# criteo-research/reco-gym

Measured on AMD Instinct MI355X. Metric: env steps/sec (organic+bandit events emitted/sec), reco-gym-v1 P=10000 K=20, higher is better.
Workload: dtype f64 (state, click, transition, policy, propensities); organic logits on MFMA as a 2-way fp16 split of fp32 operands (fp32 accumulate), every index certified against f64; 1 GPU; c3: reco-gym-v1 P=10000 K=20 sigma_omega=0.0 policy=ouc; users_per_gpu=10000000, users_total=10000000, log=16 B/row device log + float64 ps side array

## Files before the change

### recogym_amd/csrc/rg_common.hpp

```cpp

#include <hip/hip_runtime.h>

#include <cmath>
#include <cstdarg>
#include <cstdio>
#include <cstdlib>
#include <cstring>
#include <new>
#include <utility>
#include <vector>

#include "../../include/recogym_hip.h"
#include "../../include/recogym_rng.h"

#pragma once

#ifndef RG_WALK_PRECISE_CHUNK
#define RG_WALK_PRECISE_CHUNK 1
#endif

namespace rgk {

constexpr uint32_t kMaxSteps = 1u << 16;
constexpr int kBlock = 256;
// ... 210 lines not shown
    Switches w;
    const auto rd = [](const char* name) { Switch s; if (const char* e = getenv(name)) { s.set = true; s.c0 = e[0]; s.num = atoi(e); } return s; };
#define RG_SWITCH_READ(f, name) w.f = rd("RECOGYM_" name);
    RG_SWITCHES(RG_SWITCH_READ)
#undef RG_SWITCH_READ
    const char* const draws[] = {"", "f64", "fp32", "bf16", "f16"};
    if (const char* e = getenv("RECOGYM_DRAW")) for (int i = 1; i < 5; ++i) if (!strcmp(e, draws[i])) w.draw = static_cast<Switches::Draw>(i);
    if (const char* e = getenv("RECOGYM_BF16")) w.bf16_lean = !strcmp(e, "lean");
    if (const char* e = getenv("RECOGYM_REPACK_MIN")) w.repack_min = static_cast<uint64_t>(strtoull(e, nullptr, 10));
    return w;
}

struct RunOpts {
    int exact_tile;
    int exact_mix;
    int slices;
    int sweep_prefix_off;
    int debug;
    unsigned long long repack_min;
};

#define RG_LEDGER_FAMILIES(X) \
    X(draw_f64) X(draw_fp32) X(draw16_fused) X(draw16_sliced) X(search) X(draw_tp) X(pick) X(draw_cached) \
    X(sweep_xh) X(exact_m) X(exact_tile) X(exact_h) X(walk) X(walk2) X(walk_solo) \
    X(advance) X(advance_run) X(tail) X(repack) X(env0) X(logreg_screen) X(logreg_acts) X(logreg_sample) X(logreg_poly) \
    X(logreg_poly_w) X(sort_tiled) X(sort_plain) X(bayes_vb)
struct Ledger {
#define RG_LEDGER_FIELD(f) uint64_t f = 0;
    RG_LEDGER_FAMILIES(RG_LEDGER_FIELD)
#undef RG_LEDGER_FIELD
};

enum ProfClass { kProfSweep, kProfSearch , kProfResolve , kProfLogreg, kProfAdvance,
                 kProfWalk1, kProfWalk2 , kProfTail, kProfNone  };

struct WhTable {
    const double* tab;
    uint32_t n;
    uint32_t f32;
};

struct WhRun {
    WhTable wt;
    unsigned long long* rows;
    uint32_t* spill;
    uint32_t spill_cap;
};
// ... 4 lines not shown
    DevSim d;
    WhRun wh;
    RunOpts opt;
    void* workspace;
    size_t workspace_bytes;
    uint32_t t;
    uint32_t run_ahead;
    uint32_t lr_part_rows;
    uint32_t live_upper;
    bool tables_set, users_reset;
    bool repacked;
    bool walk;
    int walk_occ;
    bool walk2;
    bool walk_solo;
    int n_cus;
    int pipe_groups;
    int pipe_occ1, pipe_occ2;
    int pipe_xblocks;
    bool fin_in_sweep;
    uint32_t pipe_min_users;
    double prof_pipe_ms;
    uint32_t fate_base; const unsigned long long* fate_count;
    uint32_t repack_every;
    bool sort_plain;
    uint32_t tail_below;
    uint32_t* h_pinned;
    char* h_step;
    size_t mfma_smem, bf16_smem;
    void (*bf16_kernel)(DevSim, uint32_t, uint32_t);
    void (*xh_kernel)(DevSim, uint32_t, uint32_t);
    size_t xh_smem;
    int xh_waves;
    void (*tp_kernel)(DevSim, uint32_t, uint32_t);
    void (*pick_kernel)(DevSim, uint32_t, uint32_t);
    size_t tp_smem;
    uint32_t tp_nts;
    uint32_t sweep_lds;
    bool handover_auto;
    uint32_t draw_threads, draw_users;
    bool profiling;
    std::vector<hipEvent_t> prof_events;
    std::vector<ProfClass> prof_cls;
    size_t prof_used;
    double prof_ms[kProfNone];
    uint64_t prof_launches;
// ... 36 lines not shown
search_kernel_t logreg_acts_kernel();
search_kernel_t logreg_screen_kernel();
search_kernel_t logreg_decide_kernel();
search_kernel_t logreg_sample_kernel();
search_kernel_t poly_acts_kernel();
void (*poly_debug_kernel())(DevSim, int32_t*, uint8_t*);
search_kernel_t bayes_acts_kernel();
void (*bayes_debug_kernel())(DevSim, int32_t*, uint8_t*, double*);
void (*wh_insert_kernel())(DevSim, WhRun, uint32_t);
void (*wh_acts_kernel())(DevSim, WhRun, uint32_t, uint32_t);
void (*wh_debug_set_kernel())(DevSim, WhRun, const uint32_t*, const uint32_t*, const uint16_t*, uint32_t);
void (*wh_debug_acts_kernel())(DevSim, WhRun, const uint16_t*, int32_t*, uint8_t*, uint32_t*, uint32_t*, uint32_t*, uint32_t);
constexpr int kWhGridBlocks = 512;
advance_kernel_t advance_kernel(bool eg);
advance_run_kernel_t advance_run_kernel(bool eg);
round_rows_kernel_t round_rows_kernel();
search_kernel_t tail_kernel(bool eg);
walk_kernel_t walk_kernel_for(const DevSim& d, int occ);
walk_kernel_t walk2_kernel_for(const DevSim& d, int occ);
typedef void (*solo_kernel_t)(DevSim, uint32_t, uint32_t, uint32_t);
solo_kernel_t solo_kernel_for(const DevSim& d);
void (*cache_prefix_kernel())(DevSim, int);
void (*exact_prefix_kernel())(DevSim, uint32_t);

struct Carve {
    size_t off = 0;
    char* base;
    explicit Carve(void* b) : base(static_cast<char*>(b)) {}
    template <class T> T* take(size_t n) {
        off = align_up(off, 256);
        T* p = base ? reinterpret_cast<T*>(base + off) : nullptr;
        off += n * sizeof(T);
        return p;
    }
};

constexpr uint32_t kMaxSC = 32;
constexpr uint32_t kAhatGrid = 64;
constexpr uint32_t kHoleCode = 0xFFFFFFFFu;
#ifdef RG_WALK_TIMING
#define RG_WALK_ABL(bit) (d.ablate & (1u << (bit)))
#else
#define RG_WALK_ABL(bit) (false)
#endif

constexpr int kCntTailRows = 16, kCntTailOrganic = 17, kCntTailBandit = 18, kCntTailMaxT = 19, kCntTailTicket = 20,
              kCntTailLimit = 21, kCntWalkTicket = 22, kCntParkCnt = 23;
constexpr int kCntWalkHits = RG_CNT_MEMO_HITS;
constexpr uint32_t kMaxWalkWaves = 4096;
constexpr uint32_t kParkSlack = 2u * 64u * kMaxWalkWaves;
constexpr uint32_t kWalkCtlWords = 16;

struct Geom { uint32_t KH, KS, TP, P_pad, n_chunks, sc_chunks, n_sc, N1, N2, N3, RS, TPB, F16, XNH, XNL, XRS; bool cache, all_f64, repack, tp; };

inline bool tp_class_exists(const Geom& g) { return (g.F16 == 1 && g.KH <= 10 && g.n_chunks / 4 <= kTpBins) || g.F16 == 2; }

inline Geom geom_of(const rg_config& c, uint64_t n, const Switches& sw) {
    Geom g{};
    g.all_f64 = sw.draw == Switches::kDrawF64 || sw.force_exact.is('1');
    g.repack = n >= sw.repack_min;
    const uint32_t need = (c.K + 1) / 2;
    const uint32_t opts[] = {4, 10, 16, 32, 64};
    for (uint32_t o : opts) if (!g.KH && need <= o) g.KH = o;
    if (!g.KH) { g.all_f64 = true; return g; }
    g.KS = 2 * g.KH;
    while (g.KS % 4 != 2) ++g.KS;
    g.TP = 256;
    while (g.TP > 64 && static_cast<size_t>(g.TP) * g.KS * 4 > 24 * 1024) g.TP /= 2;
    g.P_pad = static_cast<uint32_t>(align_up(c.num_products, 256)) + 256;
    g.n_chunks = (c.num_products + 31) / 32;
    g.n_chunks = (g.n_chunks + 3) & ~3u;
    {
        const uint32_t cls[][3] = {{1, 1, 1}, {2, 1, 1}, {3, 2, 1}, {4, 3, 2}, {6, 4, 2}, {12, 8, 4}};
        for (const auto& c3 : cls)
// ... 1442 lines not shown
```

### recogym_amd/csrc/rg_host.hip

```cpp

#include "rg_common.hpp"

#ifndef RG_TP_SMEM_PAD
#define RG_TP_SMEM_PAD 0
#endif
namespace rgk {

__global__ void __launch_bounds__(kBlock) k_reset_users(DevSim d) {
    if (blockIdx.x == 0 && threadIdx.x == 0) {
        d.step_cnt[0] = d.n_users;
        d.step_cnt[1] = 0;
        d.log_base[0] = d.debug_row_base;
    }
    for (uint32_t i = blockIdx.x * kBlock + threadIdx.x; i < d.n_users; i += gridDim.x * kBlock) {
        const uint32_t user = static_cast<uint32_t>(d.first_user + i);
        if (d.env_kind) {
            const rg_u32x4 w = rg_draw(d.seed, user, 0u, 0u, RG_DRAW_RESET);
            d.pv0[i] = upper_bound_f64(d.e0_cdf_init, d.P, rg_uniform(w.w[0], w.w[1]));
        } else
        for (uint32_t j = 0; 2 * j < d.K; ++j) {
            double z0, z1;
            normal_pair(d.seed, user, 0u, j, RG_DRAW_RESET, &z0, &z1);
            d.omega[static_cast<size_t>(i) * d.OMS + 2 * j] = 0.0 + d.sigma0 * z0;
            if (2 * j + 1 < d.K) d.omega[static_cast<size_t>(i) * d.OMS + 2 * j + 1] = 0.0 + d.sigma0 * z1;
// ... 113 lines not shown
            if (which >= 2 * d.KH + 2) x = fabs(d.mu_o[p]) + x * (static_cast<double>(which - (2 * d.KH + 2) + 1) * 0.25);
        } else x = fabs(d.mu_o[p]);
        m = fmax(m, x);
    }
    red[threadIdx.x] = m;
    __syncthreads();
    for (int s2 = kBlock / 2; s2 > 0; s2 >>= 1) {
        if (threadIdx.x < s2) red[threadIdx.x] = fmax(red[threadIdx.x], red[threadIdx.x + s2]);
        __syncthreads();
    }
    if (threadIdx.x == 0) d.stats[which] = static_cast<float>(red[0] * (1.0 + 1e-6));
}

__global__ void k_tail_finish(DevSim d, uint32_t t0) {
    d.log_base[t0 + 1] = d.log_base[t0] + d.counters[kCntTailRows];
    d.step_cnt[2 * (t0 + 1)] = 0;
    d.step_cnt[2 * (t0 + 1) + 1] = 0;
}

__global__ void k_walk_finish(DevSim d) {
    d.step_cnt[0] = 0; d.step_cnt[1] = 0; d.step_cnt[2] = 0; d.step_cnt[3] = 0;
    d.log_base[0] = d.debug_row_base;
    d.log_base[1] = d.counters[kCntTailRows];
}

__global__ void k_totals(DevSim d, uint32_t t_now) {
    __shared__ unsigned long long so[kBlock], sb[kBlock];
    unsigned long long o = 0, b = 0;
    for (uint32_t t = threadIdx.x; t < t_now; t += kBlock) { o += d.step_cnt[2 * t]; b += d.step_cnt[2 * t + 1]; }
    so[threadIdx.x] = o; sb[threadIdx.x] = b;
    __syncthreads();
    for (int s = kBlock / 2; s > 0; s >>= 1) {
        if (threadIdx.x < s) { so[threadIdx.x] += so[threadIdx.x + s]; sb[threadIdx.x] += sb[threadIdx.x + s]; }
        __syncthreads();
    }
    if (threadIdx.x == 0) {
        d.counters[RG_CNT_ORGANIC] = so[0] + d.counters[kCntTailOrganic];
        d.counters[RG_CNT_BANDIT] = sb[0] + d.counters[kCntTailBandit];
        d.counters[RG_CNT_LIVE] = static_cast<unsigned long long>(d.step_cnt[2 * t_now]) + d.step_cnt[2 * t_now + 1];
        d.counters[RG_CNT_STEP] = max(static_cast<unsigned long long>(t_now), d.counters[kCntTailMaxT]);
        const unsigned long long rows = d.log_base[t_now];
        d.counters[RG_CNT_LOG_ROWS] = d.log ? (rows < d.log_cap ? rows : d.log_cap) : 0ull;
        d.counters[RG_CNT_LOG_DROPPED] = d.log ? (rows > d.log_cap ? rows - d.log_cap : 0ull) : 0ull;
    }
}

// ... 616 lines not shown
    if (int rc = prof_mark(sim, st, kProfAdvance)) return rc;
    if (d.run_ahead) {
        hipLaunchKernelGGL(advance_run_kernel(d.eg_on != 0u), dim3(grid_for(upper, kAdvBlock)), dim3(kAdvBlock), 0, st, d, t, d.run_ahead);
        sim->led.advance_run += 1;
    } else {
        hipLaunchKernelGGL(advance_kernel(d.eg_on != 0u), dim3(grid_for(upper, kAdvBlock)), dim3(kAdvBlock), 0, st, d, t, d_actions);
        sim->led.advance += 1;
    }
    if (d.sigma_omega != 0.0)
        hipLaunchKernelGGL(drift_kernel(), dim3(grid_for(static_cast<uint64_t>(upper) * ((d.K + 1) / 2))), dim3(kBlock), 0, st, d, t);
    if (d.run_ahead) hipLaunchKernelGGL(round_rows_kernel(), dim3(1), dim3(1), 0, st, d, t, 0u);
    if (sim->wh.wt.tab) {
        if (int rc = prof_mark(sim, st, kProfLogreg)) return rc;
        hipLaunchKernelGGL(wh_acts_kernel(), dim3(wh_grid(upper)), dim3(kBlock), 0, st, d, sim->wh, t, 1u);
    }
    HIP_TRY(hipGetLastError());
    if (int rc = prof_mark(sim, st, kProfNone)) return rc;
    if (sim->profiling) sim->prof_launches += 1;
    sim->t = t + 1;
    return RG_OK;
}

constexpr size_t kNoWall = ~static_cast<size_t>(0);
int close_run(rg_sim* sim, hipStream_t st, uint32_t t_end, size_t wall_from = kNoWall) {
    unsigned long long* h64 = reinterpret_cast<unsigned long long*>(sim->h_pinned);
    HIP_TRY(hipMemcpyAsync(h64, sim->d.counters + kCntTailLimit, sizeof(unsigned long long), hipMemcpyDeviceToHost, st));
    HIP_TRY(hipStreamSynchronize(st));
    if (sim->profiling && wall_from != kNoWall) {
        float ms = 0.f;
        HIP_TRY(hipEventElapsedTime(&ms, sim->prof_events[wall_from], sim->prof_events[sim->prof_used - 1]));
        sim->prof_pipe_ms += ms;
    }
    sim->t = t_end;
    sim->live_upper = 0;
    if (*h64) return fail(RG_ELIMIT, "more than %u steps", kMaxSteps);
    return RG_OK;
}

int walk_begin(rg_sim* sim, hipStream_t st) {
    (void)device_cus(sim);
    if (sim->d.debug_row_base)
        HIP_TRY(hipMemcpyAsync(sim->d.counters + kCntTailRows, &sim->d.debug_row_base, sizeof(unsigned long long), hipMemcpyHostToDevice, st));
    return RG_OK;
}
int walk_end(rg_sim* sim, hipStream_t st, size_t wall_from = kNoWall) {
    if (int rc = prof_mark(sim, st, kProfNone)) return rc;
    hipLaunchKernelGGL(k_walk_finish, dim3(1), dim3(1), 0, st, sim->d);
    HIP_TRY(hipGetLastError());
    if (int rc = prof_mark(sim, st, kProfNone)) return rc;
    if (sim->profiling) sim->prof_launches += 1;
    return close_run(sim, st, 1u, wall_from);
}

int run_walk(rg_sim* sim, hipStream_t st) {
    const DevSim& d = sim->d;
    if (int rc = walk_begin(sim, st)) return rc;
    sim->fate_count = nullptr;
    bool fused_prefix = false;
    if (int rc = prof_mark(sim, st, kProfSweep)) return rc;
    {
        DevSim ds = d;
        const auto [tiles_up, S] = sweep_slices(d.n_users, sim->draw_users, sim->opt.slices, d.n_sc);
        fused_prefix = sim->walk2 && S == 1 && f16_pipelined(sim) && !sim->opt.sweep_prefix_off;
        ds.sweep_only = fused_prefix ? 2u : 1u;
        const int grid = sweep_grid(sim, static_cast<uint64_t>(tiles_up) * S);
        hipLaunchKernelGGL(sim->bf16_kernel, dim3(grid), dim3(sim->draw_threads), sim->bf16_smem, st, ds, 0u, S);
        (S > 1 ? sim->led.draw16_sliced : sim->led.draw16_fused) += 1;
    }
    if (int rc = prof_mark(sim, st, kProfSearch)) return rc;
    hipLaunchKernelGGL(finalize_kernel_for(d), dim3(grid_for(d.n_users)), dim3(kBlock), 0, st, d);
    if (sim->walk2)
        hipLaunchKernelGGL(cache_prefix_kernel(), dim3(grid_for((static_cast<uint64_t>(d.n_users) + 7) / 8, kBlock / 64)), dim3(kBlock), 0, st, d,
                           fused_prefix ? 1 : 0);
    if (int rc = prof_mark(sim, st, kProfWalk1)) return rc;
    const size_t smem = sim->walk2 ? (kBlock / 64) * walk2_wave_lds(d.policy == RG_POLICY_ORGANIC_USER_COUNT)
                                   : (kBlock / 64) * walk_wave_lds(d.KH);
    const walk_kernel_t wk = sim->walk2 ? walk2_kernel_for(d, sim->walk_occ) : walk_kernel_for(d, d.KH <= 16 ? sim->walk_occ : 1);
    auto launch_walk = [&](uint32_t n_work, int round, uint32_t in_base, uint32_t out_base) {
        const int blocks = walk_blocks(n_work, d.KH <= 16 ? sim->walk_occ : 1, sim->n_cus);
        opt_in_lds(wk, smem);
        hipLaunchKernelGGL(wk, dim3(blocks), dim3(kBlock), smem, st, d, n_work, round, walk_chunk_rows(n_work, blocks), in_base, out_base);
        (sim->walk2 ? sim->led.walk2 : sim->led.walk) += 1;
    };
    launch_walk(d.n_users, 1, 0u, 0u);
    if (int rc = prof_mark(sim, st, kProfResolve)) return rc;
    unsigned long long* h64 = reinterpret_cast<unsigned long long*>(sim->h_pinned);
    HIP_TRY(hipMemcpyAsync(h64, d.counters + kCntParkCnt, sizeof(unsigned long long), hipMemcpyDeviceToHost, st));
    HIP_TRY(hipStreamSynchronize(st));
    const uint32_t n_park = static_cast<uint32_t>(*h64);
    if (sim->opt.debug) {
        unsigned long long ev2[2] = {0, 0};
        HIP_TRY(hipMemcpy(ev2, d.counters + kCntTailOrganic, sizeof(ev2), hipMemcpyDeviceToHost));
        fprintf(stderr, "[recogym] walk round 1: %llu organic + %llu bandit events, %u users parked of %u\n", ev2[0], ev2[1], n_park, d.n_users);
    }
    if (n_park) {
        const uint32_t mfma_of_8 = static_cast<uint32_t>(sim->opt.exact_mix);
        const exact_h_kernel_t kh = mfma_of_8 < 8 ? exact_h_kernel_for(d.XKB) : nullptr;
        const exact_m_kernel_t km = kh ? nullptr : exact_m_kernel_for(d.XKB);
        if (kh) {
            HIP_TRY(hipMemsetAsync(d.counters + kCntWalkTicket, 0, sizeof(unsigned long long), st));
            const uint32_t groups = (n_park + 255u) / 256u;
            const uint32_t grid = groups < 1024u ? groups : 1024u;
            hipLaunchKernelGGL(kh, dim3(grid), dim3(kBlock), exact_m_lds(d.XKB), st, d, n_park, mfma_of_8);
            sim->led.exact_h += 1;
        } else if (km) {
            launch_exact_m(km, d, n_park, 2, 1, n_park, st);
            sim->led.exact_m += 1;
        } else return fail(RG_ESTATE, "no float64 batch kernel for K = %u", d.K);
    }
    if (int rc = prof_mark(sim, st, kProfWalk2)) return rc;
    if (n_park) {
        const uint32_t base3 = (n_park + 63u) & ~63u;
// ... 47 lines not shown
        DevSim ds = dg;
        ds.sweep_only = 2u;
        ds.fin_in_sweep = dg.fin_in_sweep = sim->fin_in_sweep ? 1u : 0u;
        const uint32_t tiles_up = (n + sim->draw_users - 1) / sim->draw_users;
        if (int rc = prof_mark(sim, st, kProfSweep)) return rc;
        if (sim->xh_kernel) { hipLaunchKernelGGL(sim->xh_kernel, dim3(grid_for((n + 32u * sim->xh_waves - 1) / (32u * sim->xh_waves), 1)), dim3(64 * sim->xh_waves), sim->xh_smem, st, ds, 0u, 1u); sim->led.sweep_xh += 1; }
        else {
        hipLaunchKernelGGL(sim->bf16_kernel, dim3(sweep_grid(sim, tiles_up)), dim3(sim->draw_threads), sim->bf16_smem, st, ds, 0u, 1u);
        sim->led.draw16_fused += 1;
        }
        if (int rc = prof_mark(sim, st, kProfSearch)) return rc;
        hipLaunchKernelGGL(finalize_kernel_for(d), dim3(grid_for(n)), dim3(kBlock), 0, st, dg);
        hipLaunchKernelGGL(cache_prefix_kernel(), dim3(grid_for((static_cast<uint64_t>(n) + 7) / 8, kBlock / 64)), dim3(kBlock), 0, st, dg, 1);
    }
    {
        DevSim dw = dg;
        dw.q_ticket = ctl + 0; dw.q_park = ctl + 1; dw.q_count = nullptr;
        const int blocks = walk_blocks(n, sim->pipe_occ1, n_cus);
        if (int rc = prof_mark(sim, st, kProfWalk1)) return rc;
        hipLaunchKernelGGL(wk, dim3(blocks), dim3(kBlock), smem, st, dw, n, 1, walk_chunk_rows(n, blocks), 0u, region);
        sim->led.walk2 += 1;
    }
    {
        DevSim dx = dg;
        dx.q_ticket = ctl + 2; dx.q_count = ctl + 1; dx.list_in = region;
        const uint32_t est = n / 3 + 4096u;
        uint32_t xgrid = (n + 255u) / 256u;
        if (xgrid > static_cast<uint32_t>(sim->pipe_xblocks)) xgrid = static_cast<uint32_t>(sim->pipe_xblocks);
        if (int rc = prof_mark(sim, st, kProfResolve)) return rc;
        hipLaunchKernelGGL(kh, dim3(xgrid), dim3(kBlock), exact_m_lds(d.XKB), st, dx, n, mfma_of_8);
        sim->led.exact_h += 1;
        hipLaunchKernelGGL(exact_prefix_kernel(), dim3(grid_for(est, kBlock / 64)), dim3(kBlock), 0, st, dx, n);
        DevSim dr = dg;
        dr.q_ticket = ctl + 3; dr.q_park = ctl_last + 0; dr.q_count = ctl + 1;
        const int blocks = walk_blocks(est, sim->pipe_occ2, n_cus);
        if (int rc = prof_mark(sim, st, kProfWalk2)) return rc;
        hipLaunchKernelGGL(wk, dim3(blocks), dim3(kBlock), smem, st, dr, n, 2, walk_chunk_rows(est, blocks), region, base_solo);
        sim->led.walk2 += 1;
    }
    sim->fate_base = base_solo; sim->fate_count = ctl_last + 0;
    if (d.walk_handover) {
        DevSim dl = d;
        dl.q_ticket = ctl_last + 1; dl.q_count = ctl_last + 0;
        const SoloShape sh = solo_shape(n / 256u + 1024u, n_cus);
        hipLaunchKernelGGL(sk, dim3(sh.blocks), dim3(kBlock), 0, st, dl, n, sh.chunk_rows, base_solo);
        sim->led.walk_solo += 1;
    }
    return walk_end(sim, st, first_mark);
}


}

namespace {
void plan_config(rg_sim* s, const rg_config* cfg, uint64_t n_users, const Switches& w) {
    DevSim& d = s->d;
    d.P = cfg->num_products; d.K = cfg->K;
    d.seed = cfg->seed; d.policy_seed = cfg->policy_seed;
    d.cdf_o0 = cfg->trans_cdf[0][0]; d.cdf_o1 = cfg->trans_cdf[0][1];
    d.cdf_b0 = cfg->trans_cdf[1][0]; d.cdf_b1 = cfg->trans_cdf[1][1];
    d.sigma0 = cfg->sigma_omega_initial; d.sigma_omega = cfg->sigma_omega; d.change_omega_for_bandits = cfg->change_omega_for_bandits;
    d.policy = lists_unresolved(cfg->policy) ? RG_POLICY_LOGREG_FROZEN : cfg->policy;
    d.lr_poly = cfg->policy == RG_POLICY_LOGREG_POLY ? 1u : cfg->policy == RG_POLICY_BAYES_VB ? 2u : 0u;
    d.ouc_select_randomly = cfg->ouc_select_randomly; d.ouc_exploit_explore = cfg->ouc_exploit_explore;
    d.ouc_reverse_pop = cfg->ouc_reverse_pop; d.ouc_epsilon = cfg->ouc_epsilon;
    d.time_mode = cfg->time_mode; d.time_mu = cfg->time_mu; d.time_sigma = cfg->time_sigma; d.env_kind = cfg->env_kind;
    d.n_users = d.n_cap = static_cast<uint32_t>(n_users);
    d.grp_lo = 0; d.grp_n = d.n_users; d.list_in = 0;
    d.q_ticket = d.counters + kCntWalkTicket; d.q_park = d.counters + kCntParkCnt; d.q_count = nullptr;
    RunOpts& o = s->opt;
    o.exact_tile = w.exact_tile.set ? 1 : 0; o.sweep_prefix_off = w.sweep_prefix_off.set ? 1 : 0; o.debug = w.debug.set ? 1 : 0;
// ... 95 lines not shown
    s->walk_solo = !w.walk_solo.is('0');
    s->n_cus = 0;
    d.walk_refill = w.walk_refill.set ? w.walk_refill.u32() : 8;
    d.walk_handover = w.walk_handover.set ? w.walk_handover.u32() : 32;
    s->handover_auto = !w.walk_handover.set;
    d.walk_click_batch = w.walk_click_batch.set ? w.walk_click_batch.u32() : 8;
    d.walk_click_join = w.walk_click_join.is('0') ? 0 : 1;
    d.walk_helpers = w.walk_helpers.set && w.walk_helpers.u32() < kWalkHelpersMax ? w.walk_helpers.u32() : kWalkHelpersMax;
    d.walk_bias = !s->walk2 ? 8 : (d.walk_helpers ? 2 : 4);
    if (w.walk_bias.set) d.walk_bias = w.walk_bias.u32();
    d.walk_search_batch = s->walk2 && d.walk_helpers ? 24 : 16;
    if (w.walk_search_batch.set) d.walk_search_batch = w.walk_search_batch.u32() ? w.walk_search_batch.u32() : 1u;
}
void plan_pipe(rg_sim* s, const Switches& w) {
    const auto in = [](const Switch& x, int lo, int hi) { return x.set && x.num >= lo && x.num <= hi; };
    s->pipe_groups = in(w.pipe, 0, 1) ? w.pipe.num : 1;
    s->pipe_occ1 = in(w.pipe_occ1, 1, s->walk_occ) ? w.pipe_occ1.num : s->walk_occ;
    s->pipe_occ2 = in(w.pipe_occ2, 1, s->walk_occ) ? w.pipe_occ2.num : s->walk_occ;
    s->pipe_xblocks = in(w.pipe_xblocks, 1, INT_MAX) ? w.pipe_xblocks.num : 1024;
    s->pipe_min_users = in(w.pipe_min, 256, INT_MAX) ? static_cast<uint32_t>(w.pipe_min.num) : 1u << 17;
    s->fin_in_sweep = !w.fin_in_sweep.is('0');
    s->d.fin_in_sweep = 0;
    s->fate_base = 0; s->fate_count = nullptr;
}
void plan_logreg_run_ahead(rg_sim* s, const Switches& w) {
    s->run_ahead = w.run_ahead.set ? w.run_ahead.u32() : 32;
    if (s->d.lr_sample) s->run_ahead = 0;
    s->lr_part_rows = s->d.lr_part_cap;
    if (w.lr_part_cap.set && w.lr_part_cap.u32() < s->lr_part_rows) s->d.lr_part_cap = w.lr_part_cap.u32();
}
void plan_env0(rg_sim* s) {
    DevSim& d = s->d;
    if (!d.env_kind) return;
    d.use_mfma = 0; d.use_cache = 0; d.XNH = d.XNL = d.XRS = 0;
    s->bf16_kernel = nullptr; s->xh_kernel = nullptr;
    s->walk = s->walk2 = false; s->tail_below = 0; s->run_ahead = 0;
}
void plan_mfma_lds(rg_sim* s, const Switches& w) {
    if (w.lds_pad.set) s->mfma_smem += static_cast<size_t>(w.lds_pad.num);
    if (s->opt.debug && s->d.use_mfma && rg_device_count() > 0) {
        int nb = -1;
        (void)hipOccupancyMaxActiveBlocksPerMultiprocessor(&nb, reinterpret_cast<const void*>(mfma_kernel_for(10)), kBlock, s->mfma_smem);
        fprintf(stderr, "[recogym] k_draw_mfma<10>: dynamic LDS %zu B, occupancy API %d blocks/CU\n", s->mfma_smem, nb);
    }
    if (s->mfma_smem > 64 * 1024)
        for (uint32_t kh : {4u, 10u, 16u, 32u, 64u}) set_max_lds(mfma_kernel_for(kh), s->mfma_smem);
// ... 82 lines not shown
    RG_OPT("exact_mix", opt.exact_mix, int, 0, 8, true, "exact_mix must be in [0, 8]"),
    RG_OPT("slices", opt.slices, int, -1, INT64_MAX, false, "slices must be >= -1 (-1 = by population)"),
    RG_OPT("exact_tile", opt.exact_tile, int, 0, 1, false, kFlagText), RG_OPT("sweep_prefix_off", opt.sweep_prefix_off, int, 0, 1, false, kFlagText),
    RG_OPT("debug", opt.debug, int, 0, 1, false, kFlagText), RG_OPT("walk_click_join", d.walk_click_join, uint32_t, 0, 1, false, kFlagText),
    RG_OPT_U("walk_bias", d.walk_bias), RG_OPT_U("walk_refill", d.walk_refill), RG_OPT_U("walk_handover", d.walk_handover),
    RG_OPT_U("walk_click_batch", d.walk_click_batch), RG_OPT_U("walk_search_batch", d.walk_search_batch), RG_OPT_U("walk_line64", d.walk_line64),
    RG_OPT("walk_helpers", d.walk_helpers, uint32_t, 0, kWalkHelpersMax, false, "walk_helpers must be in [0, 7]"),
    RG_OPT("pipe_min_users", pipe_min_users, uint32_t, 256, INT64_MAX, false, "pipe_min_users must be >= 256"),
    RG_OPT_U("tail_below", tail_below), RG_OPT_U("repack_every", repack_every), RG_OPT_U("sweep_lds", sweep_lds),
    RG_OPT("run_ahead", run_ahead, uint32_t, 0, 64, false, "run_ahead must be <= 64 events"),
    RG_OPT_U("lr_part_cap", d.lr_part_cap),
    RG_LEDGER_FAMILIES(RG_OPT_LEDGER)
    RG_OPT_R("sweep_lds_kernel", s->tp_kernel ? 1 : 0)
    RG_OPT_R("draw_kh", s->d.KH) RG_OPT_R("draw_n1", s->d.N1) RG_OPT_R("draw_kernel", s->d.use_mfma)
    RG_OPT_R("draw_split", !s->d.N1 ? 0 : (!s->d.f16 ? 1 : (s->d.wide ? 3 : 2)))
    RG_OPT_R("draw_pipelined", (s->bf16_kernel && s->bf16_kernel == bf16p_kernel_for(s->d)) ? 1 : 0)
    RG_OPT_R("xh_waves", s->xh_kernel ? s->xh_waves : 0)
    RG_OPT_R("xh_class", s->xh_kernel ? s->d.KH * 100 + s->d.XNH * 10 + s->d.XNL : 0)
    RG_OPT_R("walk_form", !s->walk ? 0 : (s->walk2 ? 2 : 1)) RG_OPT_R("walk_occ", s->walk_occ) RG_OPT_R("walk_solo", s->walk_solo)
    RG_OPT_R("use_cache", s->d.use_cache) RG_OPT_R("fin_in_sweep", s->fin_in_sweep) RG_OPT_R("handover_auto", s->handover_auto)
    RG_OPT_R("draw_smem", s->bf16_smem) RG_OPT_R("mfma_smem", s->mfma_smem) RG_OPT_R("xh_smem", s->xh_smem) RG_OPT_R("tp_smem", s->tp_smem)
    RG_OPT_R("tp_nts", s->tp_nts) RG_OPT_R("tp_cpt", s->d.tp_cpt) RG_OPT_R("draw_threads", s->draw_threads)
    RG_OPT_R("weight_history", s->wh.wt.tab ? 1 : 0)
    RG_OPT_R("exact_rows", s->d.exact_rows) RG_OPT_R("hist_cap", s->d.hist_cap) RG_OPT_R("repack_min", s->opt.repack_min) RG_OPT_R("ablate", s->d.ablate)
};
const Option* find_option(const char* name) {
    for (const Option& o : kOptions) if (!strcmp(o.name, name)) return &o;
    return nullptr;
}
}

int rg_sim_set_option(rg_sim* sim, const char* name, int64_t value) {
    if (!sim || !name) return fail(RG_EINVAL, "NULL argument");
    const Option* o = find_option(name);
    if (!o || !o->set) return fail(RG_EINVAL, "unknown option '%s'", name);
    if (!strncmp(name, "pipe_occ", 8) && (value < 1 || value > sim->walk_occ)) return fail(RG_EINVAL, "%s must be in [1, %d]", name, sim->walk_occ);
    const bool fits = o->is_u32 ? (value >= 0 && value <= 0xFFFFFFFFll) : (value >= -2147483647 && value <= 2147483647);
    if ((value < o->lo || value > o->hi) && (fits || o->range_first)) return fail(RG_EINVAL, o->refusal, name);
    if (!fits) return fail(RG_EINVAL, o->is_u32 ? "%s must be in [0, 2^32)" : "%s out of the range of an int", name);
    if (!strcmp(name, "run_ahead") && value && sim->d.env_kind) return fail(RG_EINVAL, "env_kind 1 (reco-gym-v0) runs lock-step (run_ahead = 0)");
    if (!strcmp(name, "lr_part_cap") && static_cast<uint64_t>(value) > sim->lr_part_rows)
        return fail(RG_EINVAL, "lr_part_cap can only be lowered (the workspace holds %u rows)", sim->lr_part_rows);
    if (!strcmp(name, "walk_search_batch") && value < 1) value = 1;
    if (!strcmp(name, "walk_handover")) sim->handover_auto = false;
    o->set(sim, value);
    return RG_OK;
// ... 332 lines not shown
    if (sim->d.policy != RG_POLICY_EXTERNAL || sim->d.n_users != 1) return fail(RG_ESTATE, "rg_sim_step_user needs RG_POLICY_EXTERNAL and a one-user reset range");
    if (action < -1 || action >= static_cast<int32_t>(sim->d.P)) return fail(RG_EINVAL, "action %d is outside [0, %u) (-1: none)", action, sim->d.P);
    hipStream_t st = static_cast<hipStream_t>(stream);
    if (!sim->h_step) HIP_TRY(hipHostMalloc(reinterpret_cast<void**>(&sim->h_step), 128));
    int32_t* h_act = reinterpret_cast<int32_t*>(sim->h_step);
    *h_act = action;
    HIP_TRY(hipMemcpyAsync(sim->d.step1_buf, h_act, sizeof(int32_t), hipMemcpyHostToDevice, st));
    const uint32_t t = sim->t;
    if (int rc = launch_step(sim, reinterpret_cast<const int32_t*>(sim->d.step1_buf), st)) return rc;
    hipLaunchKernelGGL(k_step_user_pack, dim3(1), dim3(1), 0, st, sim->d, t);
    HIP_TRY(hipGetLastError());
    rg_step_result* h_res = reinterpret_cast<rg_step_result*>(sim->h_step + 64);
    HIP_TRY(hipMemcpyAsync(h_res, sim->d.step1_buf + 8, sizeof(rg_step_result), hipMemcpyDeviceToHost, st));
    HIP_TRY(hipStreamSynchronize(st));
    *out = *h_res;
    return RG_OK;
}

int rg_sim_run(rg_sim* sim, uint32_t max_steps, void* stream) {
    if (!sim) return fail(RG_EINVAL, "sim is NULL");
    if (!sim->users_reset) return fail(RG_ESTATE, "rg_sim_reset_users must be called first");
    if (sim->d.policy == RG_POLICY_EXTERNAL) return fail(RG_ESTATE, "rg_sim_run needs a device policy");
    hipStream_t st = static_cast<hipStream_t>(stream);
    if (!sim->h_pinned) HIP_TRY(hipHostMalloc(reinterpret_cast<void**>(&sim->h_pinned), 4 * sizeof(uint32_t)));
    if (sim->walk && sim->t == 0 && max_steps >= kMaxSteps) {
        const int mix = sim->opt.exact_mix;
        const bool pipe = sim->pipe_groups >= 1 && sim->walk2 && sim->walk_solo && solo_kernel_for(sim->d) && sim->d.walk_handover &&
                          f16_pipelined(sim) && sim->d.n_users >= sim->pipe_min_users &&
                          exact_h_kernel_for(sim->d.XKB) && mix < 8 && sim->opt.slices < 0 &&
                          !sim->opt.sweep_prefix_off;
        return pipe ? run_walk_pipe(sim, st) : run_walk(sim, st);
    }
    if (sim->t == 0 && max_steps >= kMaxSteps && sim->run_ahead && !sim->d.change_omega_for_bandits && !sim->d.use_cache && !sim->d.u_override &&
        !sim->wh.wt.tab) {
        sim->d.run_ahead = sim->run_ahead;
        hipLaunchKernelGGL(round_rows_kernel(), dim3(1), dim3(1), 0, st, sim->d, 0u, 1u);
    }
    uint32_t done_steps = 0;
    const uint32_t chunk = 16;
    while (done_steps < max_steps) {
        const uint32_t todo = (max_steps - done_steps) < chunk ? (max_steps - done_steps) : chunk;
        for (uint32_t i = 0; i < todo; ++i)
            if (int rc = launch_step(sim, nullptr, st)) return rc;
        done_steps += todo;
        HIP_TRY(hipMemcpyAsync(sim->h_pinned, sim->d.step_cnt + 2 * sim->t, 2 * sizeof(uint32_t),
                               hipMemcpyDeviceToHost, st));
        HIP_TRY(hipStreamSynchronize(st));
// ... 293 lines not shown
```

### recogym_amd/csrc/rg_walk.hip

```cpp

#include "rg_common.hpp"

namespace rgk {

template <int KH, int OCC, bool DENSE>
__global__ void __launch_bounds__(kBlock, OCC) k_walk(DevSim d_arg, uint32_t n_work, int round, uint32_t chunk_rows,
                                                       uint32_t in_base, uint32_t out_base) {
    (void)d_arg;
    const __attribute__((address_space(4))) char* kargs =
        (const __attribute__((address_space(4))) char*)__builtin_amdgcn_kernarg_segment_ptr();
    const DevSim& d = *(const DevSim*)kargs;
    constexpr int K2 = 2 * KH;
    constexpr bool kPreciseChunk = RG_WALK_PRECISE_CHUNK && KH <= 10;
    constexpr double kLog2e64 = 1.4426950408889634074;
    constexpr int kEmpty = 3;
    constexpr int kPhantom = 4;
    extern __shared__ __attribute__((aligned(16))) char smem_raw[];
    const int wave = threadIdx.x >> 6, lane = lane_id();
    constexpr int kIdle = 5;
    char* wbase = smem_raw + static_cast<size_t>(wave) * walk_wave_lds(KH);
    float* om32 = reinterpret_cast<float*>(wbase);
    double* mbox = reinterpret_cast<double*>(om32 + kWalkUsers * K2 * 64);
    uint32_t* slots = reinterpret_cast<uint32_t*>(mbox + 64 * 3);
    const uint32_t n_cc = d.PT / 64;
// ... 559 lines not shown
    if (hit) v = ccstar * 64 + static_cast<uint32_t>(__builtin_ctzll(hit));
    return v;
}

__global__ void __launch_bounds__(kBlock) k_exact_prefix(DevSim d, uint32_t n_list) {
    const int lane = lane_id();
    const uint32_t n_cc = d.PT / 64;
    const uint32_t waves = gridDim.x * (kBlock / 64);
    if (d.q_count) n_list = static_cast<uint32_t>(*d.q_count);
    for (uint32_t w = blockIdx.x * (kBlock / 64) + (threadIdx.x >> 6); w < n_list; w += waves) {
        const uint32_t slot = d.park_list[d.list_in + w];
        if (slot == 0xFFFFFFFFu) continue;
        double* row = d.exact_sums + static_cast<size_t>(slot) * n_cc;
        double run = 0.0;
        for (uint32_t c0 = 0; c0 < n_cc; c0 += 64) {
            const uint32_t c = c0 + lane;
            const double incl = wave_scan(c < n_cc ? row[c] : 0.0, lane);
            if (c < n_cc) row[c] = run + incl;
            run += __shfl(incl, 63);
        }
    }
}

__device__ __forceinline__ uint32_t exact_pick_call(const DevSim& d, const double* sums, const double* om, double M,
                                                   double u, int lane) {
    return exact_pick_wave(d, sums, om, M, u, 1u, lane);
}

constexpr uint32_t kHcLine = 32;

template <int KH, int HIST>
__global__ void __launch_bounds__(kBlock, (KH <= 10 ? 3 : 2)) k_walk2(DevSim d_arg, uint32_t n_work, int round, uint32_t chunk_rows,
                                                        uint32_t in_base, uint32_t out_base) {
    (void)d_arg;
    const __attribute__((address_space(4))) char* kargs =
        (const __attribute__((address_space(4))) char*)__builtin_amdgcn_kernarg_segment_ptr();
    constexpr int K2 = 2 * KH;
    constexpr bool kPreciseChunk = RG_WALK_PRECISE_CHUNK && KH <= 10;
    constexpr double kLog2e64 = 1.4426950408889634074;
    constexpr int KC = ((K2 + 3) / 4) * 4;
    constexpr int kEmpty = 3, kPhantom = 4;
    extern __shared__ __attribute__((aligned(16))) char smem_raw[];
    const int wave = threadIdx.x >> 6, lane = lane_id();
    char* wbase = smem_raw + static_cast<size_t>(wave) * walk2_wave_lds(HIST);
    hent_t* hl = reinterpret_cast<hent_t*>(wbase) + lane;
    float* mboxf = reinterpret_cast<float*>(wbase + (HIST ? 16 * 64 * 8 : 0));
// ... 78 lines not shown
                asm volatile("" ::: "memory");
            }
        };
        {
            unsigned long long dead = __ballot(st == kEmpty);
            if (dead && !exhausted && (static_cast<uint32_t>(__popcll(dead)) >= d.walk_refill || dead == ~0ull)) {
                flush_hist(st == kEmpty && hdirty);
                hdirty = hdirty && st != kEmpty;
                for (int pass = 0; pass < 2 && dead; ++pass) {
                    if (res_next == res_end) {
                        if (exhausted) break;
                        uint32_t base = 0;
                        if (lane == 0) base = static_cast<uint32_t>(atomicAdd(d.q_ticket, 64ull));
                        base = __builtin_amdgcn_readfirstlane(base);
                        if (base >= n_work) { exhausted = true; break; }
                        res_next = base; res_end = min(base + 64u, n_work);
                    }
                    const uint32_t take = min(static_cast<uint32_t>(__popcll(dead)), res_end - res_next);
                    const uint32_t r = prefix_in_mask(dead);
                    const bool mine = ((dead >> lane) & 1ull) != 0 && r < take;
                    if (mine) {
                        const uint32_t idx = res_next + r;
                        uint32_t s2 = d.grp_lo + idx;
                        if (round >= 2) s2 = d.park_list[in_base + idx];
                        if (s2 != 0xFFFFFFFFu) {
                            slot = s2; st = kWSlow; t = 0u; pend = false; hdirty = false;
                            if (round >= 2) {
                                const uint32_t pt = d.park_t[s2];
                                t = pt & 0xFFFFFFu; st = static_cast<int>((pt >> 24) & 7u); pend = (pt >> 27) & 1u;
                                if (round == 2) d.f64_valid[s2] = 1;
                                if (pend) st = kWSlow;
                            }
                            {
                                const float4* rp = reinterpret_cast<const float4*>(d.cache_row + static_cast<size_t>(s2) * d.cache_row_f);
#pragma unroll
                                for (int k4 = 0; k4 < K2 / 4; ++k4) {
                                    const float4 x = rp[11 + k4];
                                    om[4 * k4] = x.x; om[4 * k4 + 1] = x.y; om[4 * k4 + 2] = x.z; om[4 * k4 + 3] = x.w;
                                }
#pragma unroll
                                for (int k = (K2 / 4) * 4; k < K2; ++k) om[k] = reinterpret_cast<const float*>(rp)[44 + k];
                            }
                            if (HIST == 2) load_compact(s2);
                            else
                            if (HIST) {
                                const ulonglong2* hr2 = reinterpret_cast<const ulonglong2*>(hist_row(d, s2));
#pragma unroll
// ... 1159 lines not shown
        default: return ouc ? k_walk_solo<16, 1> : k_walk_solo<16, 0>;
    }
#endif
}
walk_kernel_t walk2_kernel_for(const DevSim& d, int occ) {
    const bool ouc = d.policy == RG_POLICY_ORGANIC_USER_COUNT;
    if (d.KH > 16 || !d.walk_hot) return nullptr;
    if (ouc && !(d.ouc_exploit_explore && d.ouc_epsilon == 0.0 && d.ouc_select_randomly)) return nullptr;
    if (d.policy != RG_POLICY_UNIFORM_ENV && d.policy != RG_POLICY_RANDOM_AGENT && d.policy != RG_POLICY_LAST_VIEW_TABLE && !ouc) return nullptr;
#ifdef RG_W2_ONLY
    return k_walk2<10, 2>;
#else
    (void)occ;
    const bool compact = ouc && d.P <= 65535u && d.hist_cap >= 32u && d.hist_cap <= 32768u && !d.walk_line64;
    switch (d.KH) {
        case 4: return ouc ? (compact ? k_walk2<4, 2> : k_walk2<4, 1>) : k_walk2<4, 0>;
        case 10: return ouc ? (compact ? k_walk2<10, 2> : k_walk2<10, 1>) : k_walk2<10, 0>;
        default: return ouc ? (compact ? k_walk2<16, 2> : k_walk2<16, 1>) : k_walk2<16, 0>;
    }
#endif
}
void (*cache_prefix_kernel())(DevSim, int) { return k_cache_prefix; }
void (*exact_prefix_kernel())(DevSim, uint32_t) { return k_exact_prefix; }

walk_kernel_t walk_kernel_for(const DevSim& d, int occ) {
#ifdef RG_W2_ONLY
    return nullptr;
#else
    const bool dense = d.policy == RG_POLICY_ORGANIC_USER_COUNT && !(d.ouc_exploit_explore && d.ouc_epsilon == 0.0);
#define RG_W(kh, o) (dense ? k_walk<kh, o, true> : k_walk<kh, o, false>)
    switch (d.KH) {
        case 4: return RG_W(4, 3);
        case 10: return RG_W(10, 3);
        case 16: return RG_W(16, 3);
        default: return RG_W(32, 1);
    }
#undef RG_W
#endif
}

}

#ifdef RG_WALK_TIMING
extern "C" void rg_debug_walk_kinds(unsigned long long* out, int clear) {
    (void)hipDeviceSynchronize();
    (void)hipMemcpyFromSymbol(out, HIP_SYMBOL(rgk::g_walk_stat), sizeof(unsigned long long) * 20);
// ... 4 lines not shown
```

Measured before the change: 9.851 billion events/s.

## Compact park list into dense exact list before second walk round

Adds a park-compaction kernel that squeezes hole entries out of the park list into a dense exact_list, using per-block prefix scans and atomic reservations. It also counts how many parked users still have pending handover. The exact-prefix and round-2 walk kernels then read the dense list and its count instead of the sparse park region, so fewer queue tickets are spent on empty slots. The cost is an extra kernel launch, an extra pass over the list, and a wider readback of counters at walk end for the new stats options.

```diff
diff --git a/recogym_amd/csrc/rg_common.hpp b/recogym_amd/csrc/rg_common.hpp
--- a/recogym_amd/csrc/rg_common.hpp
+++ b/recogym_amd/csrc/rg_common.hpp
@@ -256,7 +256,7 @@
 
 #define RG_LEDGER_FAMILIES(X) \
     X(draw_f64) X(draw_fp32) X(draw16_fused) X(draw16_sliced) X(search) X(draw_tp) X(pick) X(draw_cached) \
-    X(sweep_xh) X(exact_m) X(exact_tile) X(exact_h) X(walk) X(walk2) X(walk_solo) \
+    X(sweep_xh) X(exact_m) X(exact_tile) X(exact_h) X(walk) X(walk2) X(walk_solo) X(park_compact) \
     X(advance) X(advance_run) X(tail) X(repack) X(env0) X(logreg_screen) X(logreg_acts) X(logreg_sample) X(logreg_poly) \
     X(logreg_poly_w) X(sort_tiled) X(sort_plain) X(bayes_vb)
 struct Ledger {
@@ -307,6 +307,7 @@
     uint32_t pipe_min_users;
     double prof_pipe_ms;
     uint32_t fate_base; const unsigned long long* fate_count;
+    int64_t park_slots, park_users, handed_over, batch_users;
     uint32_t repack_every;
     bool sort_plain;
     uint32_t tail_below;
@@ -389,6 +390,7 @@
 solo_kernel_t solo_kernel_for(const DevSim& d);
 void (*cache_prefix_kernel())(DevSim, int);
 void (*exact_prefix_kernel())(DevSim, uint32_t);
+void (*park_compact_kernel())(DevSim);
 
 struct Carve {
     size_t off = 0;
@@ -417,6 +419,9 @@
 constexpr uint32_t kMaxWalkWaves = 4096;
 constexpr uint32_t kParkSlack = 2u * 64u * kMaxWalkWaves;
 constexpr uint32_t kWalkCtlWords = 16;
+constexpr uint32_t kCtlAll = 4, kCtlHanded = 5, kCtlLimit = 6;
+constexpr uint32_t kDenseList = 0xFFFFFFFFu;
+constexpr uint32_t kCompactTile = 4096;
 
 struct Geom { uint32_t KH, KS, TP, P_pad, n_chunks, sc_chunks, n_sc, N1, N2, N3, RS, TPB, F16, XNH, XNL, XRS; bool cache, all_f64, repack, tp; };
 
diff --git a/recogym_amd/csrc/rg_host.hip b/recogym_amd/csrc/rg_host.hip
--- a/recogym_amd/csrc/rg_host.hip
+++ b/recogym_amd/csrc/rg_host.hip
@@ -159,6 +159,7 @@
     d.step_cnt[0] = 0; d.step_cnt[1] = 0; d.step_cnt[2] = 0; d.step_cnt[3] = 0;
     d.log_base[0] = d.debug_row_base;
     d.log_base[1] = d.counters[kCntTailRows];
+    d.walk_ctl[kCtlLimit] = d.counters[kCntTailLimit];
 }
 
 __global__ void k_totals(DevSim d, uint32_t t_now) {
@@ -821,10 +822,12 @@
 }
 
 constexpr size_t kNoWall = ~static_cast<size_t>(0);
-int close_run(rg_sim* sim, hipStream_t st, uint32_t t_end, size_t wall_from = kNoWall) {
+constexpr size_t kPinnedWords = 8;
+int close_run(rg_sim* sim, hipStream_t st, uint32_t t_end, size_t wall_from = kNoWall, const unsigned long long* from = nullptr, size_t words = 1) {
     unsigned long long* h64 = reinterpret_cast<unsigned long long*>(sim->h_pinned);
-    HIP_TRY(hipMemcpyAsync(h64, sim->d.counters + kCntTailLimit, sizeof(unsigned long long), hipMemcpyDeviceToHost, st));
+    HIP_TRY(hipMemcpyAsync(h64, from ? from : sim->d.counters + kCntTailLimit, sizeof(unsigned long long) * words, hipMemcpyDeviceToHost, st));
     HIP_TRY(hipStreamSynchronize(st));
+    h64 += words - 1;
     if (sim->profiling && wall_from != kNoWall) {
         float ms = 0.f;
         HIP_TRY(hipEventElapsedTime(&ms, sim->prof_events[wall_from], sim->prof_events[sim->prof_used - 1]));
@@ -842,19 +845,30 @@
         HIP_TRY(hipMemcpyAsync(sim->d.counters + kCntTailRows, &sim->d.debug_row_base, sizeof(unsigned long long), hipMemcpyHostToDevice, st));
     return RG_OK;
 }
-int walk_end(rg_sim* sim, hipStream_t st, size_t wall_from = kNoWall) {
+int walk_end(rg_sim* sim, hipStream_t st, size_t wall_from = kNoWall, bool dense = false) {
     if (int rc = prof_mark(sim, st, kProfNone)) return rc;
     hipLaunchKernelGGL(k_walk_finish, dim3(1), dim3(1), 0, st, sim->d);
     HIP_TRY(hipGetLastError());
     if (int rc = prof_mark(sim, st, kProfNone)) return rc;
     if (sim->profiling) sim->prof_launches += 1;
-    return close_run(sim, st, 1u, wall_from);
+    if (!dense) return close_run(sim, st, 1u, wall_from);
+    static_assert(kCtlLimit <= kPinnedWords, "walk_ctl's words 1 .. kCtlLimit fit the pinned staging");
+    const int rc = close_run(sim, st, 1u, wall_from, sim->d.walk_ctl + 1, kCtlLimit);
+    const unsigned long long* h64 = reinterpret_cast<const unsigned long long*>(sim->h_pinned);
+    if (rc == RG_OK || rc == RG_ELIMIT) {
+        sim->park_slots = static_cast<int64_t>(h64[0]);
+        sim->batch_users = static_cast<int64_t>(h64[kCtlAll - 1]);
+        sim->handed_over = static_cast<int64_t>(h64[kCtlHanded - 1]);
+        sim->park_users = sim->batch_users - sim->handed_over;
+    }
+    return rc;
 }
 
 int run_walk(rg_sim* sim, hipStream_t st) {
     const DevSim& d = sim->d;
     if (int rc = walk_begin(sim, st)) return rc;
     sim->fate_count = nullptr;
+    sim->park_slots = sim->batch_users = 0; sim->park_users = sim->handed_over = -1;
     bool fused_prefix = false;
     if (int rc = prof_mark(sim, st, kProfSweep)) return rc;
     {
@@ -887,6 +901,7 @@
     HIP_TRY(hipMemcpyAsync(h64, d.counters + kCntParkCnt, sizeof(unsigned long long), hipMemcpyDeviceToHost, st));
     HIP_TRY(hipStreamSynchronize(st));
     const uint32_t n_park = static_cast<uint32_t>(*h64);
+    sim->park_slots = sim->batch_users = n_park;
     if (sim->opt.debug) {
         unsigned long long ev2[2] = {0, 0};
         HIP_TRY(hipMemcpy(ev2, d.counters + kCntTailOrganic, sizeof(ev2), hipMemcpyDeviceToHost));
@@ -980,8 +995,17 @@
         sim->led.walk2 += 1;
     }
     {
+        DevSim dc = dg;
+        dc.list_in = region;
+        uint32_t cgrid = (n + kParkSlack + kCompactTile - 1) / kCompactTile;
+        if (cgrid > 1024u) cgrid = 1024u;
+        if (int rc = prof_mark(sim, st, kProfResolve)) return rc;
+        hipLaunchKernelGGL(park_compact_kernel(), dim3(cgrid), dim3(kBlock), 0, st, dc);
+        sim->led.park_compact += 1;
+    }
+    {
         DevSim dx = dg;
-        dx.q_ticket = ctl + 2; dx.q_count = ctl + 1; dx.list_in = region;
+        dx.q_ticket = ctl + 2; dx.q_count = ctl + kCtlAll; dx.park_list = d.exact_list; dx.list_in = 0;
         const uint32_t est = n / 3 + 4096u;
         uint32_t xgrid = (n + 255u) / 256u;
         if (xgrid > static_cast<uint32_t>(sim->pipe_xblocks)) xgrid = static_cast<uint32_t>(sim->pipe_xblocks);
@@ -990,10 +1014,10 @@
         sim->led.exact_h += 1;
         hipLaunchKernelGGL(exact_prefix_kernel(), dim3(grid_for(est, kBlock / 64)), dim3(kBlock), 0, st, dx, n);
         DevSim dr = dg;
-        dr.q_ticket = ctl + 3; dr.q_park = ctl_last + 0; dr.q_count = ctl + 1;
+        dr.q_ticket = ctl + 3; dr.q_park = ctl_last + 0; dr.q_count = ctl + kCtlAll;
         const int blocks = walk_blocks(est, sim->pipe_occ2, n_cus);
         if (int rc = prof_mark(sim, st, kProfWalk2)) return rc;
-        hipLaunchKernelGGL(wk, dim3(blocks), dim3(kBlock), smem, st, dr, n, 2, walk_chunk_rows(est, blocks), region, base_solo);
+        hipLaunchKernelGGL(wk, dim3(blocks), dim3(kBlock), smem, st, dr, n, 2, walk_chunk_rows(est, blocks), kDenseList, base_solo);
         sim->led.walk2 += 1;
     }
     sim->fate_base = base_solo; sim->fate_count = ctl_last + 0;
@@ -1004,7 +1028,7 @@
         hipLaunchKernelGGL(sk, dim3(sh.blocks), dim3(kBlock), 0, st, dl, n, sh.chunk_rows, base_solo);
         sim->led.walk_solo += 1;
     }
-    return walk_end(sim, st, first_mark);
+    return walk_end(sim, st, first_mark, true);
 }
 
 
@@ -1146,6 +1170,7 @@
     s->fin_in_sweep = !w.fin_in_sweep.is('0');
     s->d.fin_in_sweep = 0;
     s->fate_base = 0; s->fate_count = nullptr;
+    s->park_slots = s->park_users = s->handed_over = s->batch_users = 0;
 }
 void plan_logreg_run_ahead(rg_sim* s, const Switches& w) {
     s->run_ahead = w.run_ahead.set ? w.run_ahead.u32() : 32;
@@ -1274,6 +1299,7 @@
     RG_OPT_R("draw_smem", s->bf16_smem) RG_OPT_R("mfma_smem", s->mfma_smem) RG_OPT_R("xh_smem", s->xh_smem) RG_OPT_R("tp_smem", s->tp_smem)
     RG_OPT_R("tp_nts", s->tp_nts) RG_OPT_R("tp_cpt", s->d.tp_cpt) RG_OPT_R("draw_threads", s->draw_threads)
     RG_OPT_R("weight_history", s->wh.wt.tab ? 1 : 0)
+    RG_OPT_R("park_slots", s->park_slots) RG_OPT_R("park_users", s->park_users) RG_OPT_R("handed_over", s->handed_over) RG_OPT_R("batch_users", s->batch_users)
     RG_OPT_R("exact_rows", s->d.exact_rows) RG_OPT_R("hist_cap", s->d.hist_cap) RG_OPT_R("repack_min", s->opt.repack_min) RG_OPT_R("ablate", s->d.ablate)
 };
 const Option* find_option(const char* name) {
@@ -1652,7 +1678,7 @@
     if (!sim->users_reset) return fail(RG_ESTATE, "rg_sim_reset_users must be called first");
     if (sim->d.policy == RG_POLICY_EXTERNAL) return fail(RG_ESTATE, "rg_sim_run needs a device policy");
     hipStream_t st = static_cast<hipStream_t>(stream);
-    if (!sim->h_pinned) HIP_TRY(hipHostMalloc(reinterpret_cast<void**>(&sim->h_pinned), 4 * sizeof(uint32_t)));
+    if (!sim->h_pinned) HIP_TRY(hipHostMalloc(reinterpret_cast<void**>(&sim->h_pinned), kPinnedWords * sizeof(unsigned long long)));
     if (sim->walk && sim->t == 0 && max_steps >= kMaxSteps) {
         const int mix = sim->opt.exact_mix;
         const bool pipe = sim->pipe_groups >= 1 && sim->walk2 && sim->walk_solo && solo_kernel_for(sim->d) && sim->d.walk_handover &&
diff --git a/recogym_amd/csrc/rg_walk.hip b/recogym_amd/csrc/rg_walk.hip
--- a/recogym_amd/csrc/rg_walk.hip
+++ b/recogym_amd/csrc/rg_walk.hip
@@ -605,6 +605,51 @@
     }
 }
 
+__global__ void __launch_bounds__(kBlock) k_park_compact(DevSim d) {
+    constexpr int kPer = kCompactTile / kBlock;
+    __shared__ uint32_t s_wave[kBlock / 64];
+    __shared__ uint32_t s_base;
+    const int lane = lane_id(), wave = threadIdx.x >> 6;
+    const uint32_t n = static_cast<uint32_t>(d.walk_ctl[1]);
+    const uint32_t* src = d.park_list + d.list_in;
+    for (uint32_t t0 = blockIdx.x * kCompactTile; t0 < n; t0 += gridDim.x * kCompactTile) {
+        uint32_t slot[kPer];
+        uint32_t n_u = 0u, n_h = 0u;
+#pragma unroll
+        for (int j = 0; j < kPer; ++j) {
+            const uint32_t idx = t0 + threadIdx.x * static_cast<uint32_t>(kPer) + static_cast<uint32_t>(j);
+            slot[j] = idx < n ? src[idx] : 0xFFFFFFFFu;
+        }
+#pragma unroll
+        for (int j = 0; j < kPer; ++j)
+            if (slot[j] != 0xFFFFFFFFu) {
+                n_u += 1u;
+                n_h += ((d.park_t[slot[j]] >> 27) & 1u) ^ 1u;
+            }
+        const uint32_t mine = n_u | (n_h << 16);
+        uint32_t incl = mine;
+        for (int o = 1; o < 64; o <<= 1) {
+            const uint32_t y = static_cast<uint32_t>(__shfl_up(static_cast<int>(incl), o));
+            if (lane >= o) incl += y;
+        }
+        __syncthreads();
+        if (lane == 63) s_wave[wave] = incl;
+        __syncthreads();
+        uint32_t before = 0u, total = 0u;
+#pragma unroll
+        for (int w = 0; w < kBlock / 64; ++w) { if (w < wave) before += s_wave[w]; total += s_wave[w]; }
+        if (threadIdx.x == 0) {
+            s_base = (total & 0xFFFFu) ? static_cast<uint32_t>(atomicAdd(d.walk_ctl + kCtlAll, static_cast<unsigned long long>(total & 0xFFFFu))) : 0u;
+            if (total >> 16) atomicAdd(d.walk_ctl + kCtlHanded, static_cast<unsigned long long>(total >> 16));
+        }
+        __syncthreads();
+        uint32_t at = s_base + ((before + incl - mine) & 0xFFFFu);
+#pragma unroll
+        for (int j = 0; j < kPer; ++j)
+            if (slot[j] != 0xFFFFFFFFu) d.exact_list[at++] = slot[j];
+    }
+}
+
 __device__ __forceinline__ uint32_t exact_pick_call(const DevSim& d, const double* sums, const double* om, double M,
                                                    double u, int lane) {
     return exact_pick_wave(d, sums, om, M, u, 1u, lane);
@@ -729,7 +774,10 @@
                     if (mine) {
                         const uint32_t idx = res_next + r;
                         uint32_t s2 = d.grp_lo + idx;
-                        if (round >= 2) s2 = d.park_list[in_base + idx];
+                        if (round >= 2) {
+                            const uint32_t* lst = in_base == kDenseList ? d.exact_list : d.park_list + in_base;
+                            s2 = lst[idx];
+                        }
                         if (s2 != 0xFFFFFFFFu) {
                             slot = s2; st = kWSlow; t = 0u; pend = false; hdirty = false;
                             if (round >= 2) {
@@ -1935,6 +1983,7 @@
 }
 void (*cache_prefix_kernel())(DevSim, int) { return k_cache_prefix; }
 void (*exact_prefix_kernel())(DevSim, uint32_t) { return k_exact_prefix; }
+void (*park_compact_kernel())(DevSim) { return k_park_compact; }
 
 walk_kernel_t walk_kernel_for(const DevSim& d, int occ) {
 #ifdef RG_W2_ONLY
```

New measurement: 10.02 billion events/s (median of 6 runs). 1.7% higher.
